# GreenleafLab/NucleoATAC

Measured on AMD Instinct MI355X. Metric: Mbp/s through occ+nuc signal pipeline, higher is better.
Workload: dtype f64

## Files before the change

nucleoatac_amd/csrc/natac_api.hip:

```cpp
#include "../../include/natac.h"
#ifndef NATAC_GNBL
#define NATAC_GNBL 2
#endif
#include "natac_kernels.hpp"
#include "natac_fft_bg.hpp"
#include "natac_occ_fast.hpp"
#include "natac_cand.hpp"
#include "natac_covsweep.hpp"
#include "natac_textz.hpp"
#include "natac_cores.hpp"
#include "natac_writer.hpp"
#include "natac_tabix.hpp"
#include "natac_pack.hpp"
#include "natac_bam.hpp"
#include "natac_bam_dev.hpp"
#include "natac_fragfile.hpp"
#include "natac_fragfile_dev.hpp"
#include "natac_fasta.hpp"
#include "natac_fuzzfit.hpp"
#include "natac_bedtab.hpp"
#include "natac_runtime.hpp"
#include "natac_pwmfit.hpp"
#include "natac_sites.hpp"
#include "natac_cellcounts.hpp"
// ... 149 lines not shown
    if (!count) return fail(NATAC_E_ARG, "count is NULL");
    int n = 0;
    hipError_t e = hipGetDeviceCount(&n);
    if (e != hipSuccess) {
        *count = 0;
        return fail(NATAC_E_HIP, "hipGetDeviceCount: %s", hipGetErrorString(e));
    }
    *count = n;
    return NATAC_OK;
}

int natac_ctx_create(int device_id, natac_ctx **out) {
    if (!out) return fail(NATAC_E_ARG, "out is NULL");
    *out = nullptr;
    int n = 0;
    HIPCHK(hipGetDeviceCount(&n));
    if (device_id < 0 || device_id >= n) return fail(NATAC_E_ARG, "device %d out of range (%d devices)", device_id, n);
    HIPCHK(hipSetDevice(device_id));
    natac_ctx *c = new natac_ctx();
    c->device = device_id;
    HIPCHK(hipGetDeviceProperties(&c->prop, device_id));
    HIPCHK(hipStreamCreateWithFlags(&c->stream, hipStreamNonBlocking));
    HIPCHK(hipEventCreate(&c->t0));
    HIPCHK(hipEventCreate(&c->t1));
    {
        const char *e = getenv("NATAC_BG_DIRECT");
        c->bg_direct = e && e[0] == '1';
        e = getenv("NATAC_BG_EXT");
        c->bg_ext = !(e && e[0] == '0');
        e = getenv("NATAC_OCC_GENERAL");
        c->occ_force_general = e && e[0] == '1';
        e = getenv("NATAC_OCC_ORDER");
        c->occ_ordered = !(e && e[0] == '0');
    }
    *out = c;
    return NATAC_OK;
}

void natac_ctx_destroy(natac_ctx *c) {
    if (!c) return;
    (void)hipSetDevice(c->device);
    (void)sync_all(c);
    prof_collect(c);
    if (c->t0) (void)hipEventDestroy(c->t0);
    if (c->t1) (void)hipEventDestroy(c->t1);
    if (c->ck_stream) (void)hipStreamDestroy(c->ck_stream);
    if (c->ck_start) (void)hipEventDestroy(c->ck_start);
    if (c->d_ck) (void)hipFree(c->d_ck);
    if (c->copy_stream) (void)hipStreamDestroy(c->copy_stream);
    if (c->stream) (void)hipStreamDestroy(c->stream);
    delete c;
}

int natac_ctx_sync(natac_ctx *c) {
    if (!c) return fail(NATAC_E_ARG, "ctx is NULL");
    HIPCHK(hipSetDevice(c->device));
    HIPCHK(sync_all(c));
    prof_collect(c);
    return NATAC_OK;
}

int natac_ctx_device_info(natac_ctx *c, char *name, size_t name_len, int *n_cu, size_t *mem_bytes) {
    if (!c) return fail(NATAC_E_ARG, "ctx is NULL");
    if (name && name_len) {
        snprintf(name, name_len, "%s (%s)", c->prop.name, c->prop.gcnArchName);
    }
// ... 234 lines not shown
        std::vector<double> tw(2 * (size_t)natac::FFT_N);
        for (int k = 0; k < natac::FFT_N; ++k) {
            const double a = 2.0 * M_PI * k / natac::FFT_N;
            tw[2 * k] = std::cos(a);
            tw[2 * k + 1] = -std::sin(a);
        }
        if (const char *e = getenv("NATAC_FAULT_TWIDDLE")) {
            int k = 0; double dlt = 0.0;
            if (sscanf(e, "%d:%lf", &k, &dlt) == 2 && k >= 0 && k < natac::FFT_N) tw[2 * (size_t)k] += dlt;
        }
        if ((rc = dev_upload(c, c->d_fft_tw, tw.data(), tw.size()))) return rc;
        HIPCHK(sync_all(c));
    }
    if (!c->fft_dirty) return NATAC_OK;
    HIPCHK(sync_all(c));
    const int npair = (c->R + 1) / 2;
    if ((rc = dev_alloc(c->d_fft_k, (size_t)npair * 2 * natac::FFT_N))) return rc;
    hipLaunchKernelGGL(natac_fft_template, dim3(npair), dim3(64), 0, c->stream, c->d_vmat, c->d_srow, c->R, c->W, c->d_fft_tw, c->d_fft_k);
    if (c->W >= natac::FFT_EXT) {
        c->d_fft_mtab.reset(); c->d_fft_swt.reset();
        const int NJ = (c->R + 3) / 4;
        if ((rc = dev_alloc(c->d_fft_mtab, (size_t)2 * NJ * 64)) || (rc = dev_alloc(c->d_fft_swt, (size_t)4 * NJ))) return rc;
        hipLaunchKernelGGL(natac_fft_edge_table_mfma, dim3((2 * NJ * 64 + 255) / 256), dim3(256), 0, c->stream, c->d_vmat, c->d_srow, c->R, c->W, NJ,
                           c->d_fft_mtab, c->d_fft_swt);
    }
    HIPCHK(hipGetLastError());
    c->fft_dirty = false;
    return NATAC_OK;
}

static int ensure_window(natac_ctx *c, PoolBuf<double> &slot, int *slotM, double *slotsd, int M, double sd, double *slotsum = nullptr) {
    if (slot && *slotM == M && *slotsd == sd) return NATAC_OK;
    HIPCHK(sync_all(c));
    std::vector<double> w((size_t)M);
    for (int i = 0; i < M; ++i) {
        double n = (double)i - (M - 1) / 2.0;
        double q = n / sd;
        w[i] = std::exp(-0.5 * (q * q));
    }
    int rc = dev_upload(c, slot, w.data(), (size_t)M);
    if (rc) return rc;
    HIPCHK(sync_all(c));
    if (slotsum) {
        double acc = 0.0;
        for (int i = 0; i < M; ++i) acc = acc + w[i];
        *slotsum = acc;
    }
    *slotM = M;
    *slotsd = sd;
    return NATAC_OK;
}

static int run_exp_bias(natac_batch *b, hipStream_t st, bool from_occ) {
    if (!b->d_bias) return NATAC_OK;
    if (from_occ && b->ebias_fresh) { b->ebias_fresh = false; return NATAC_OK; }
    b->ebias_fresh = !from_occ;
    int rc;
    if (!b->d_ebias && (rc = dev_alloc(b->d_ebias, (size_t)b->nb))) return rc;
    const int blocks = (int)std::min<long long>((b->nb + 255) / 256, 16384);
    hipLaunchKernelGGL(natac_exp_bias, dim3(blocks), dim3(256), 0, st, b->d_bias, b->d_ebias, b->nb);
    return NATAC_OK;
}

static ChunkTable make_table(natac_batch *b) {
    ChunkTable t;
    t.nc = b->nc; t.chunk_len = b->d_len; t.frag_off = b->d_frag_off; t.lpos = b->d_lpos; t.ilen = b->d_ilen;
    t.centre = b->d_centre; t.bias_off = b->d_bias_off; t.bias = b->d_bias; t.ebias = b->d_ebias; t.bias_left = b->bias_left;
    t.bias_right = b->bias_right; t.out_off = b->d_out_off; t.grid_off = b->d_grid_off;
    return t;
}
static VMatDev make_vmat(natac_ctx *c) {
    VMatDev v;
    v.mat = c->d_vmat; v.matp = c->d_vmat_pad; v.srow = c->d_srow; v.lower = c->vlower; v.upper = c->vupper; v.w = c->vw; v.R = c->R; v.W = c->W;
// ... 135 lines not shown
    delete b;
}

int natac_batch_release_outputs(natac_batch *b) {
    if (!b) return fail(NATAC_E_ARG, "batch is NULL");
    natac_ctx *c = b->ctx;
    HIPCHK(hipSetDevice(c->device));
    HIPCHK(sync_all(c));
    prof_collect(c);
    for (auto &t : b->d_track) t.reset();
    for (auto &g : b->d_grid) g.reset();
    b->d_bnum.reset(); b->d_bcov.reset(); b->d_gsum.reset(); b->d_pk_out.reset();
    b->d_pk_chunk.reset(); b->d_pk_pos.reset(); b->d_opk_vals.reset(); b->d_opk_keep.reset(); b->d_nuc_dist.reset();
    b->d_fmt_out.reset(); b->fmt_bytes = -1;
    (void)fmt_pending_wait(b);
    b->pk_cap = 0; b->pk_n = -1; b->opk_cap = 0; b->opk_n = -1;
    b->out = BatchOutputs();
    HIPCHK(hipMemsetAsync(b->d_status, 0, (size_t)b->nc * sizeof(int), c->stream));
    HIPCHK(hipStreamSynchronize(c->stream));
    return NATAC_OK;
}

int natac_batch_info(natac_batch *b, int64_t *total_bp, int64_t *total_grid, int64_t *n_frags) {
    if (!b) return fail(NATAC_E_ARG, "batch is NULL");
    if (total_bp) *total_bp = b->total_bp;
    if (total_grid) *total_grid = b->total_grid;
    if (n_frags) *n_frags = b->nf;
    return NATAC_OK;
}

static int ensure_track(natac_batch *b, int t) {
    if (b->d_track[t]) return NATAC_OK;
    return dev_alloc(b->d_track[t], (size_t)b->total_bp);
}

int natac_run_nuc(natac_batch *b, double smooth_sd) {
    if (!b) return fail(NATAC_E_ARG, "batch is NULL");
    natac_ctx *c = b->ctx;
    HIPCHK(hipSetDevice(c->device));
    int rc = ensure_srow(c);
    if (rc) return rc;
    if (!(smooth_sd > 0)) return fail(NATAC_E_ARG, "smooth_sd must be positive");
    const int M = 6 * (int)smooth_sd + 1;
    const int need_l = c->vw + ((c->vupper - 2) >> 1), need_r = c->vw + ((c->vupper - 1) >> 1) + 1;
    if (b->d_bias && (b->bias_left < need_l || b->bias_right < need_r))
        return fail(NATAC_E_ARG, "bias track must extend >= %d left / %d right of the chunk (has %d / %d)", need_l, need_r,
                    b->bias_left, b->bias_right);
    for (int i = 0; i < b->nc; ++i)
        if (b->h_len[i] < M) return fail(NATAC_E_ARG, "chunk %d shorter (%d) than the smoothing window (%d)", i, b->h_len[i], M);
    if ((rc = ensure_window(c, c->d_win_nuc, &c->win_nuc_M, &c->win_nuc_sd, M, smooth_sd, &c->win_nuc_sum))) return rc;
    const bool use_fft = fft_bg_applicable(c);
    for (int t : {NATAC_T_NUC_COV, NATAC_T_NFR_COV, NATAC_T_RAW, NATAC_T_NORM, NATAC_T_SMOOTH})
        if ((rc = ensure_track(b, t))) return rc;
    if (!use_fft && (rc = ensure_track(b, NATAC_T_BACKGROUND))) return rc;
    if (!b->d_bnum && (rc = dev_alloc(b->d_bnum, (size_t)b->total_bp))) return rc;
    if (!b->d_bcov && (rc = dev_alloc(b->d_bcov, (size_t)b->total_bp))) return rc;
    const bool fast = !use_fft && (c->W == 121 && c->vlower >= 2);
    if (use_fft) {
        if ((rc = ensure_fft(c))) return rc;
        const int TV = FFT_N - c->W + 1;
        const bool ext_ok = bg_ext_possible(c);
        const int key = -(TV + (ext_ok ? 4096 : 0));
        if (b->bgG != key) {
            if ((rc = build_tiles_bg(b, TV, ext_ok))) return rc;
            b->bgG = key;
        }
    } else if (fast) {
        const int G = choose_bg_G(b, c->W);
        if (G != b->bgG) {
            if ((rc = build_tiles(b, 64 * G, b->d_tiles_bg, &b->n_tiles_bg))) return rc;
            b->bgG = G;
        }
    }
    if (!b->d_ebias && b->d_bias && (rc = dev_alloc(b->d_ebias, (size_t)b->nb))) return rc;
    const ChunkTable ct = make_table(b);
    const VMatDev vm = make_vmat(c);
    natac_ctx::Ev ev;
    if (!b->d_ranges256 && (rc = dev_alloc(b->d_ranges256, (size_t)b->n_tiles256))) return rc;
    if ((M - 1) / 2 == 30 && !b->d_tiles1k && (rc = build_tiles(b, 1024, b->d_tiles1k, &b->n_tiles1k))) return rc;
    prof_begin(c, NATAC_K_FRAG_GATHER, ev);
    if (b->ranges256_w != c->vw) {
        hipLaunchKernelGGL(natac_tile_ranges256, dim3((b->n_tiles256 + 255) / 256), dim3(256), 0, c->stream, ct, b->d_tiles256,
                           b->n_tiles256, c->vw, b->d_ranges256);
        b->ranges256_w = c->vw;
    }
    const bool cov_mine = b->out.occ_cov_by_nuc && b->out.nuc_w == c->vw && b->out.nuc_upper == c->vupper;
    const bool cov_too = c->have_occ && c->flank == c->vw && c->occ_upper == c->vupper &&
                         (b->out.track[NATAC_T_OCC_COV] == TS_EMPTY || cov_mine);
    if (cov_too && (rc = ensure_track(b, NATAC_T_OCC_COV))) return rc;
    constexpr int GNBL = NATAC_GNBL;
    hipLaunchKernelGGL((natac_frag_gather<GNBL>), dim3(b->n_tiles256), dim3(256 / GNBL), 0, c->stream, ct, b->d_tiles256, b->d_ranges256, vm,
                       b->d_track[NATAC_T_NUC_COV], b->d_track[NATAC_T_NFR_COV], b->d_track[NATAC_T_RAW],
                       cov_too ? b->d_track[NATAC_T_OCC_COV] : nullptr);
    prof_end(c, ev);
    prof_begin(c, NATAC_K_BACKGROUND, ev);
    if ((rc = run_exp_bias(b, c->stream, false))) return rc;
    if (use_fft) {
        const size_t lds = bg_fft_lds_bytes(vm.upper);
        hipLaunchKernelGGL(natac_background_fft, dim3(b->n_tiles_bg), dim3(64), lds, c->stream, ct, b->d_tiles_bg, vm, c->d_fft_tw,
                           c->d_fft_k, b->d_track[NATAC_T_NUC_COV], b->d_track[NATAC_T_RAW], (double *)nullptr,
                           b->d_track[NATAC_T_NORM], b->d_bnum, b->d_bcov, (unsigned)b->n_tiles_bg, c->d_fft_mtab,
                           c->d_fft_swt, (c->R + 3) / 4);
    } else if (fast) {
        switch (b->bgG) {
            case 7: launch_bg<7>(b, ct, vm); break;
            case 9: launch_bg<9>(b, ct, vm); break;
            case 13: launch_bg<13>(b, ct, vm); break;
            default: launch_bg<17>(b, ct, vm); break;
        }
    } else {
        hipLaunchKernelGGL(natac_background_generic, dim3(b->n_tiles256), dim3(256), 0, c->stream, ct, b->d_tiles256, vm,
                           b->d_track[NATAC_T_NUC_COV], b->d_track[NATAC_T_RAW], b->d_track[NATAC_T_BACKGROUND],
                           b->d_track[NATAC_T_NORM], b->d_bnum, b->d_bcov);
    }
    prof_end(c, ev);
    prof_begin(c, NATAC_K_SMOOTH_NUC, ev);
    {
        const int h = (M - 1) / 2;
        if (h == 30) {
            hipLaunchKernelGGL((natac_smooth_same4<true, 30>), dim3(b->n_tiles1k), dim3(256), (size_t)8 * SM4_S(30) * sizeof(double),
                               c->stream, ct, b->d_tiles1k, c->d_win_nuc, c->win_nuc_sum, b->d_track[NATAC_T_NORM],
                               b->d_track[NATAC_T_SMOOTH]);
        } else {
            const size_t lds = ((size_t)2 * (256 + 2 * h)) * sizeof(double);
            hipLaunchKernelGGL((natac_smooth_same<true>), dim3(b->n_tiles256), dim3(256), lds, c->stream, ct, b->d_tiles256,
                               c->d_win_nuc, M, c->win_nuc_sum, b->d_track[NATAC_T_NORM], b->d_track[NATAC_T_SMOOTH]);
        }
    }
    prof_end(c, ev);
    HIPCHK(hipGetLastError());
    for (int t : {NATAC_T_NUC_COV, NATAC_T_NFR_COV, NATAC_T_RAW, NATAC_T_NORM, NATAC_T_SMOOTH}) b->out.track[t] = TS_RUN;
    b->out.track[NATAC_T_BACKGROUND] = use_fft ? TS_PENDING : TS_RUN;
    b->out.bg_gen = c->model_gen;
    b->out.nuc_w = c->vw;
    b->out.nuc_lower = c->vlower;
    b->out.nuc_upper = c->vupper;
    b->out.occ_cov_by_nuc = cov_too;
    return NATAC_OK;
}

static void launch_occ_smooth_generic(natac_batch *b, const ChunkTable &ct, const OccModelDev &om, int M, double *dst_occ, double *dst_lo,
                                      double *dst_hi) {
    natac_ctx *c = b->ctx;
    const int h = (M - 1) / 2;
    const int NB = 2 * ((h + c->step - 1) / c->step) + 2, NG = (255 + 2 * h) / c->step + 3;
    const size_t lds = ((size_t)((M + 1) & ~1) + (size_t)c->step * NB + 3 * (size_t)NG) * sizeof(double);
    hipLaunchKernelGGL(natac_occ_smooth, dim3(b->n_tiles256), dim3(256), lds, c->stream, ct, b->d_tiles256, om, c->d_win_occ, M,
                       b->d_grid[0], b->d_grid[1], b->d_grid[2], dst_occ, dst_lo, dst_hi);
}

static int occ_smooth_blocks(int h, int step) {
    if (h % step == 0) return 2 * (h / step) + 2;
    return (h + step - 1) / step + (h + step - 1) / step + 1;
}

static int ensure_block_weights(natac_ctx *c, int M, double sd, int NB) {
    if (c->d_wb_occ && c->wb_M == M && c->wb_step == c->step) return NATAC_OK;
    HIPCHK(sync_all(c));
    const int h = (M - 1) / 2, step = c->step;
    std::vector<double> w((size_t)M), wb((size_t)step * NB + step);
    for (int i = 0; i < M; ++i) {
        const double n = (double)i - (M - 1) / 2.0, q = n / sd;
        w[i] = std::exp(-0.5 * (q * q));
    }
// ... 12 lines not shown
        for (int bi = 0; bi < NB; ++bi) den = std::fma(wb[(size_t)bi * step + j], 1.0, den);
        wb[(size_t)NB * step + j] = den;
    }
    int rc = dev_upload(c, c->d_wb_occ, wb.data(), wb.size());
    if (rc) return rc;
    HIPCHK(sync_all(c));
    c->wb_M = M;
    c->wb_step = step;
    return NATAC_OK;
}

static int materialise_bg(natac_batch *b) {
    natac_ctx *c = b->ctx;
    int rc = ensure_track(b, NATAC_T_BACKGROUND);
    if (rc) return rc;
    const int blocks = (int)std::min<long long>((b->total_bp + 255) / 256, 1 << 20);
    hipLaunchKernelGGL(natac_bg_from_factors, dim3(blocks), dim3(256), 0, c->stream, b->d_bnum, b->d_track[NATAC_T_NUC_COV], b->d_bcov,
                       b->d_track[NATAC_T_BACKGROUND], b->total_bp);
    HIPCHK(hipGetLastError());
    b->out.track[NATAC_T_BACKGROUND] = TS_RUN;
    return NATAC_OK;
}

static int materialise_prefill(natac_batch *b) {
    natac_ctx *c = b->ctx;
    int rc = ensure_track(b, NATAC_T_OCC_PREFILL);
    if (rc) return rc;
    if ((rc = ensure_window(c, c->d_win_occ, &c->win_occ_M, &c->win_occ_sd, 2 * c->flank + 1, c->flank / 3.0))) return rc;
    const ChunkTable ct = make_table(b);
    const OccModelDev om = make_occ(c);
    launch_occ_smooth_generic(b, ct, om, 2 * c->flank + 1, b->d_track[NATAC_T_OCC_PREFILL], nullptr, nullptr);
    HIPCHK(hipGetLastError());
    b->out.track[NATAC_T_OCC_PREFILL] = TS_RUN;
    return NATAC_OK;
}

static int need_track(natac_batch *b, int t) {
    static const char *const names[NATAC_T_COUNT] = {"NUC_COV", "NFR_COV", "RAW", "BACKGROUND", "NORM", "SMOOTH", "OCC", "OCC_LOWER",
                                                     "OCC_UPPER", "OCC_COV", "INS", "OCC_PREFILL", "INS_SMOOTH", "CENTER_COV", "BIAS"};
    if (t < 0 || t >= NATAC_T_COUNT) return fail(NATAC_E_ARG, "bad track id %d", t);
    if (b->out.track[t] == TS_EMPTY)
        return fail(NATAC_E_STATE, "track NATAC_T_%s holds nothing: no stage has written it and natac_batch_set_track has not", names[t]);
    if (b->out.track[t] != TS_PENDING) return NATAC_OK;
    if (t == NATAC_T_OCC_PREFILL) {
        const int rc = need_occ_geometry(b, "NATAC_T_OCC_PREFILL");
        if (rc) return rc;
    }
    HIPCHK(hipSetDevice(b->ctx->device));
    return t == NATAC_T_BACKGROUND ? materialise_bg(b) : materialise_prefill(b);
}

static int occ_prepare(natac_batch *b) {
    if (!b) return fail(NATAC_E_ARG, "batch is NULL");
    natac_ctx *c = b->ctx;
    HIPCHK(hipSetDevice(c->device));
    if (!c->have_occ) return fail(NATAC_E_STATE, "natac_set_occ_model has not been called");
    const int M = 2 * c->flank + 1;
    const double sd = c->flank / 3.0;
    const int need_l = c->flank + ((c->occ_upper - 2) >> 1), need_r = c->flank + ((c->occ_upper - 1) >> 1) + 1;
    if (b->d_bias && (b->bias_left < need_l || b->bias_right < need_r))
        return fail(NATAC_E_ARG, "bias track must extend >= %d left / %d right of the chunk (has %d / %d)", need_l, need_r,
                    b->bias_left, b->bias_right);
    for (int i = 0; i < b->nc; ++i)
        if (b->h_len[i] < M) return fail(NATAC_E_ARG, "chunk %d shorter (%d) than the occupancy window (%d)", i, b->h_len[i], M);
    int rc;
    if ((rc = ensure_window(c, c->d_win_occ, &c->win_occ_M, &c->win_occ_sd, M, sd))) return rc;
    if (!b->d_grid_off || b->grid_step != c->step) {
        b->h_grid_off.assign((size_t)b->nc + 1, 0);
        for (int i = 0; i < b->nc; ++i) {
            const int nk = (b->h_len[i] > c->halfstep) ? (b->h_len[i] - c->halfstep + c->step - 1) / c->step : 0;
            b->h_grid_off[i + 1] = b->h_grid_off[i] + nk;
        }
        b->total_grid = b->h_grid_off[b->nc];
        HIPCHK(sync_all(c));
        b->out.grids = false;
        if (b->out.track[NATAC_T_OCC_PREFILL] == TS_PENDING) b->out.track[NATAC_T_OCC_PREFILL] = TS_EMPTY;
        if ((rc = dev_upload(c, b->d_grid_off, b->h_grid_off.data(), (size_t)b->nc + 1))) return rc;
        for (auto &g : b->d_grid)
            if ((rc = dev_alloc(g, (size_t)b->total_grid))) return rc;
        if ((rc = build_tiles(b, OCC_T * OCC_NP, b->d_tiles_occ, &b->n_tiles_occ, true, c->step, c->halfstep))) return rc;
        b->d_ranges_occ.reset(); b->d_order_occ.reset();
// ... 384 lines not shown
        if (dc.ok()) {
            if (mode == 1)
                hipLaunchKernelGGL(natac_cov_literal_many, dim3(NBLK, (unsigned)m), dim3(256), 0, c->stream, d_p, c->d_vmat, N, d_out);
            else if (mode == 0)
                hipLaunchKernelGGL((natac_cov_closed_many<double>), dim3((unsigned)m), dim3(256), 0, c->stream, d_p, c->d_vmat, N, d_out);
            else
                hipLaunchKernelGGL((natac_cov_closed_many<float>), dim3((unsigned)m), dim3(256), 0, c->stream, d_p, c->d_vmat, N, d_out);
            dc.launched();
        }
        dc.fetch(part.data(), d_out, (size_t)m * per);
        if ((rc = dc.sync())) return rc;
        for (int64_t k = 0; k < m; ++k) {
            double s = 0;
            for (int j = 0; j < per; ++j) s += part[(size_t)k * per + j];
            var[k0 + k] = s;
        }
    }
    std::vector<double> reads((size_t)n_cand);
    std::vector<long long> idx((size_t)n_cand);
    for (int64_t k = 0; k < n_cand; ++k) idx[(size_t)k] = b->h_out_off[cand_chunk[k]] + cand_pos[k];
    const long long *d_idx = dc.upload(idx.data(), (size_t)n_cand);
    double *d_r = dc.alloc<double>((size_t)n_cand);
    if (dc.ok()) {
        hipLaunchKernelGGL(natac_gather_f64, dim3((unsigned)((n_cand + 255) / 256)), dim3(256), 0, c->stream,
                           b->d_track[NATAC_T_NUC_COV], d_idx, (long long)n_cand, d_r);
        dc.launched();
    }
    dc.fetch(reads.data(), d_r, (size_t)n_cand);
    if ((rc = dc.finish())) return rc;
    for (int64_t k = 0; k < n_cand; ++k) var[k] = var[k] * cov_reads(reads[(size_t)k]);
    return NATAC_OK;
}

static int run_peaks_impl(natac_batch *b, const double *sig_a, const double *sig_b, bool with_stats, double min_signal, int sep,
                          int boundary, int order, const double *jitter, int64_t n_jitter, int64_t *n_cand) {
    if (!b || !jitter || !n_cand) return fail(NATAC_E_ARG, "null argument");
    natac_ctx *c = b->ctx;
    if (order < 1 || order > 255 || sep < 1 || boundary < 0) return fail(NATAC_E_ARG, "bad peak parameters");
    int maxL = 0;
    for (int i = 0; i < b->nc; ++i) maxL = std::max(maxL, b->h_len[i]);
    if (n_jitter < maxL) return fail(NATAC_E_ARG, "jitter stream (%lld) shorter than the longest chunk (%d)", (long long)n_jitter, maxL);
    HIPCHK(hipSetDevice(c->device));
    HIPCHK(sync_all(c));
    int rc;
    if (with_stats && (rc = ensure_srow(c))) return rc;
    if (!b->d_jitter || b->n_jitter < maxL) {
        if ((rc = dev_upload(c, b->d_jitter, jitter, (size_t)maxL))) return rc;
        HIPCHK(hipStreamSynchronize(c->stream));
        b->n_jitter = maxL;
    } else {
        HIPCHK(hipMemcpyAsync(b->d_jitter, jitter, (size_t)maxL * sizeof(double), hipMemcpyHostToDevice, c->stream));
        HIPCHK(hipStreamSynchronize(c->stream));
    }
    if (b->pk_order != order) {
        std::vector<long long> cap((size_t)b->nc + 1, 0);
        for (int i = 0; i < b->nc; ++i) cap[i + 1] = cap[i] + b->h_len[i] / (order + 1) + 2;
        b->slot_total = cap[b->nc];
        b->d_cap_off.reset(); b->d_slot.reset();
        if ((rc = dev_upload(c, b->d_cap_off, cap.data(), (size_t)b->nc + 1))) return rc;
        HIPCHK(hipStreamSynchronize(c->stream));
        if ((rc = dev_alloc(b->d_slot, (size_t)b->slot_total))) return rc;
        b->pk_order = order;
    }
    if (!b->d_pk_count && (rc = dev_alloc(b->d_pk_count, (size_t)b->nc))) return rc;
    if (!b->d_pk_offs && (rc = dev_alloc(b->d_pk_offs, (size_t)b->nc + 1))) return rc;
    const ChunkTable ct = make_table(b);
    const double *norm = sig_a, *sm = sig_b;
    natac_ctx::Ev ev;
    prof_begin(c, NATAC_K_CAND, ev);
    hipLaunchKernelGGL(natac_status_clear, dim3((b->nc + 255) / 256), dim3(256), 0, c->stream, b->d_status, b->nc, 2);
    {
        const int pk_cap = (std::min(PEAK_MAX, maxL / (order + 1) + 2) + 7) & ~7;
        const size_t lds_lists = (size_t)pk_cap * (sizeof(double) + sizeof(int) + 1);
        const int bt = maxL <= 4096 ? 256 : 1024;
        const int nj = (maxL + bt - 1) / bt;
        const size_t lds_reg = (size_t)((bt * nj + 2 * order + 1) & ~1) * sizeof(double) + lds_lists;
#define NATAC_PEAKS_REG(NJ, BT)                                                                                                    \
    case NJ: {                                                                                                                     \
        auto kfn = natac_peaks_chunk_reg<NJ, BT>;                                                                                  \
        if (lds_reg > 64 * 1024) HIPCHK(hipFuncSetAttribute((const void *)kfn, hipFuncAttributeMaxDynamicSharedMemorySize, (int)lds_reg)); \
        hipLaunchKernelGGL(kfn, dim3(b->nc), dim3(BT), lds_reg, c->stream, ct, norm, sm, b->d_jitter, min_signal, boundary, order, sep, \
                           pk_cap, b->d_cap_off, b->d_slot, b->d_pk_count, b->d_status);                                          \
        break;                                                                                                                     \
    }
        if (bt == 256) {
            switch (nj) {
                NATAC_PEAKS_REG(1, 256) NATAC_PEAKS_REG(2, 256) NATAC_PEAKS_REG(3, 256) NATAC_PEAKS_REG(4, 256) NATAC_PEAKS_REG(5, 256)
                NATAC_PEAKS_REG(6, 256) NATAC_PEAKS_REG(7, 256) NATAC_PEAKS_REG(8, 256) NATAC_PEAKS_REG(9, 256) NATAC_PEAKS_REG(10, 256)
                NATAC_PEAKS_REG(11, 256) NATAC_PEAKS_REG(12, 256) NATAC_PEAKS_REG(13, 256) NATAC_PEAKS_REG(14, 256)
                NATAC_PEAKS_REG(15, 256) NATAC_PEAKS_REG(16, 256)
            }
        } else if (nj <= 16 && lds_reg <= 150 * 1024) {
            switch (nj) {
                NATAC_PEAKS_REG(5, 1024) NATAC_PEAKS_REG(6, 1024) NATAC_PEAKS_REG(7, 1024) NATAC_PEAKS_REG(8, 1024) NATAC_PEAKS_REG(9, 1024)
                NATAC_PEAKS_REG(10, 1024) NATAC_PEAKS_REG(11, 1024) NATAC_PEAKS_REG(12, 1024) NATAC_PEAKS_REG(13, 1024)
                NATAC_PEAKS_REG(14, 1024) NATAC_PEAKS_REG(15, 1024) NATAC_PEAKS_REG(16, 1024)
            }
        } else {
            const int seg = 4096;
            const size_t lds = (size_t)((seg + 2 * order + 1) & ~1) * sizeof(double) + lds_lists;
            double *big_sig = nullptr;
            int *big_pos = nullptr;
            unsigned char *big_state = nullptr;
            if (maxL / (order + 1) + 2 > pk_cap) {
                if (b->d_pk_big.size() < (size_t)b->slot_total * 2 + 2 && (rc = dev_alloc(b->d_pk_big, (size_t)b->slot_total * 2 + 2)))
                    return rc;
                big_sig = b->d_pk_big;
                big_pos = (int *)(b->d_pk_big + b->slot_total);
                big_state = (unsigned char *)(big_pos + b->slot_total);
            }
            hipLaunchKernelGGL(natac_peaks_chunk, dim3(b->nc), dim3(256), lds, c->stream, ct, norm, sm, b->d_jitter, min_signal,
                               boundary, order, sep, seg, pk_cap, b->d_cap_off, b->d_slot, b->d_pk_count, b->d_status, big_sig, big_pos,
                               big_state);
        }
#undef NATAC_PEAKS_REG
    }
    hipLaunchKernelGGL(natac_scan_counts, dim3(1), dim3(1024), 0, c->stream, b->d_pk_count, b->nc, b->d_pk_offs);
    long long total = 0;
    HIPCHK(hipGetLastError());
    HIPCHK(hipMemcpyAsync(&total, b->d_pk_offs + b->nc, sizeof(long long), hipMemcpyDeviceToHost, c->stream));
    HIPCHK(hipStreamSynchronize(c->stream));
    if (total > b->pk_cap) {
        b->d_pk_chunk.reset(); b->d_pk_pos.reset(); b->d_pk_out.reset();
        b->pk_cap = 0;
        const long long cap = total + total / 4 + 16;
        if ((rc = dev_alloc(b->d_pk_chunk, (size_t)cap)) || (rc = dev_alloc(b->d_pk_pos, (size_t)cap)) ||
            (rc = dev_alloc(b->d_pk_out, (size_t)3 * cap))) {
            b->d_pk_chunk.reset(); b->d_pk_pos.reset();
            return rc;
        }
        b->pk_cap = cap;
    }
    if (total > 0) {
        hipLaunchKernelGGL(natac_compact_candidates, dim3((b->nc + 3) / 4), dim3(256), 0, c->stream, b->nc, b->d_pk_count, b->d_pk_offs,
                           b->d_cap_off, b->d_slot, b->d_pk_chunk, b->d_pk_pos);
        if (with_stats) {
            const VMatDev vm = make_vmat(c);
            launch_candidates(c, ct, vm, b->d_pk_chunk, b->d_pk_pos, total, b->d_track[NATAC_T_NUC_COV], b->d_track[NATAC_T_NORM],
                              b->out.bg_gen == c->model_gen ? b->d_bnum : nullptr, b->out.bg_gen == c->model_gen ? b->d_bcov : nullptr,
                              b->d_pk_out, b->d_pk_out + b->pk_cap, b->d_pk_out + 2 * b->pk_cap,
                              b->ranges256_w == c->vw ? b->d_tile256_first : nullptr, b->ranges256_w == c->vw ? b->d_ranges256 : nullptr);
        }
    }
    b->pk_has_stats = with_stats;
    prof_end(c, ev);
    HIPCHK(hipGetLastError());
    b->pk_n = total;
    *n_cand = total;
    return NATAC_OK;
}

int natac_run_peaks(natac_batch *b, double min_signal, int sep, int boundary, int order, const double *jitter, int64_t n_jitter,
                    int64_t *n_cand) {
    if (!b) return fail(NATAC_E_ARG, "batch is NULL");
    int rc;
    if ((rc = need_track(b, NATAC_T_SMOOTH)) || (rc = need_candidate_inputs(b)) || (rc = need_nuc_geometry(b, "natac_run_peaks"))) return rc;
    return run_peaks_impl(b, b->d_track[NATAC_T_NORM], b->d_track[NATAC_T_SMOOTH], true, min_signal, sep, boundary, order, jitter,
                          n_jitter, n_cand);
}

int natac_run_track_peaks(natac_batch *b, int track, double min_signal, int sep, int boundary, int order, const double *jitter,
                          int64_t n_jitter, int64_t *n_peaks) {
    if (!b) return fail(NATAC_E_ARG, "batch is NULL");
    if (track == NATAC_T_INS) return fail(NATAC_E_ARG, "peak search needs a float64 track");
    int rc = need_track(b, track);
    if (rc) return rc;
    return run_peaks_impl(b, b->d_track[track], nullptr, false, min_signal, sep, boundary, order, jitter, n_jitter, n_peaks);
}

int natac_run_occ_peaks(natac_batch *b, double min_occ, int sep, const double *jitter, int64_t n_jitter, int64_t *n_peaks) {
    if (!b || !n_peaks) return fail(NATAC_E_ARG, "null argument");
    int rc;
    for (int t : {NATAC_T_OCC, NATAC_T_OCC_LOWER, NATAC_T_OCC_UPPER, NATAC_T_OCC_COV}) if ((rc = need_track(b, t))) return rc;
    if ((rc = need_occ_geometry(b, "natac_run_occ_peaks"))) return rc;
    natac_ctx *c = b->ctx;
    const int U = c->occ_upper;
    if (U > 1024) return fail(NATAC_E_ARG, "upper > 1024");
    rc = run_peaks_impl(b, b->d_track[NATAC_T_OCC], nullptr, false, min_occ, sep, sep / 2, 1, jitter, n_jitter, n_peaks);
    if (rc) return rc;
    const long long n = *n_peaks;
    if (n > b->opk_cap || !b->d_opk_vals) {
        if (n > b->opk_cap) HIPCHK(sync_all(c));
        const long long cap = n > b->opk_cap ? n + n / 4 + 16 : 16;
        b->d_opk_vals.reset(); b->d_opk_keep.reset();
        b->opk_cap = 0;
        if ((rc = dev_alloc(b->d_opk_vals, (size_t)4 * cap)) || (rc = dev_alloc(b->d_opk_keep, (size_t)cap))) {
            b->d_opk_vals.reset();
            return rc;
        }
        b->opk_cap = cap;
    }
// ... 72 lines not shown
int natac_batch_download(natac_batch *b, int track, void *dst, size_t dst_bytes) {
    if (!b || !dst) return fail(NATAC_E_ARG, "null argument");
    int rc = need_track(b, track);
    if (rc) return rc;
    const size_t need = (size_t)b->total_bp * (track == NATAC_T_INS ? sizeof(int) : sizeof(double));
    if (dst_bytes != need) return fail(NATAC_E_ARG, "destination holds %zu bytes, track needs %zu", dst_bytes, need);
    HIPCHK(hipSetDevice(b->ctx->device));
    HIPCHK(hipMemcpyAsync(dst, b->d_track[track], need, hipMemcpyDeviceToHost, b->ctx->stream));
    HIPCHK(sync_all(b->ctx));
    prof_collect(b->ctx);
    return NATAC_OK;
}

int natac_batch_download_grid(natac_batch *b, int which, double *dst, size_t dst_bytes) {
    if (!b || !dst) return fail(NATAC_E_ARG, "null argument");
    if (which < 0 || which > 2) return fail(NATAC_E_ARG, "bad grid id");
    if (!b->out.grids) return fail(NATAC_E_STATE, "natac_run_occ has not run");
    const size_t need = (size_t)b->total_grid * sizeof(double);
    if (dst_bytes != need) return fail(NATAC_E_ARG, "destination holds %zu bytes, grid needs %zu", dst_bytes, need);
    HIPCHK(hipSetDevice(b->ctx->device));
    HIPCHK(hipMemcpyAsync(dst, b->d_grid[which], need, hipMemcpyDeviceToHost, b->ctx->stream));
    HIPCHK(sync_all(b->ctx));
    return NATAC_OK;
}

int natac_batch_set_track(natac_batch *b, int track, const double *vals, size_t n) {
    if (!b || !vals) return fail(NATAC_E_ARG, "null argument");
    if (track < 0 || track >= NATAC_T_COUNT || track == NATAC_T_INS) return fail(NATAC_E_ARG, "bad track id %d (float64 tracks only)", track);
    if (n != (size_t)b->total_bp) return fail(NATAC_E_ARG, "track needs %lld values, got %zu", b->total_bp, n);
    natac_ctx *c = b->ctx;
    HIPCHK(hipSetDevice(c->device));
    int rc;
    if (track == NATAC_T_NUC_COV && b->out.track[NATAC_T_BACKGROUND] == TS_PENDING && (rc = materialise_bg(b))) return rc;
    HIPCHK(sync_all(c));
    if ((rc = ensure_track(b, track))) return rc;
    HIPCHK(hipMemcpyAsync(b->d_track[track], vals, n * sizeof(double), hipMemcpyHostToDevice, c->stream));
    HIPCHK(hipStreamSynchronize(c->stream));
    b->out.track[track] = TS_HOST;
    if (track == NATAC_T_OCC_COV) b->out.occ_cov_by_nuc = false;
    return NATAC_OK;
}

int natac_batch_status(natac_batch *b, int32_t *dst, size_t dst_bytes) {
    if (!b || !dst) return fail(NATAC_E_ARG, "null argument");
    if (dst_bytes != (size_t)b->nc * sizeof(int)) return fail(NATAC_E_ARG, "status buffer must hold n_chunks int32");
    HIPCHK(hipSetDevice(b->ctx->device));
    HIPCHK(hipMemcpyAsync(dst, b->d_status, dst_bytes, hipMemcpyDeviceToHost, b->ctx->stream));
    HIPCHK(sync_all(b->ctx));
    return NATAC_OK;
}

int natac_batch_track_ptr(natac_batch *b, int track, void **dptr) {
    if (!b || !dptr) return fail(NATAC_E_ARG, "null argument");
    if (track < 0 || track >= NATAC_T_COUNT) return fail(NATAC_E_ARG, "bad track id");
    *dptr = nullptr;
    if (b->out.track[track] == TS_EMPTY) return NATAC_OK;
    int rc = need_track(b, track);
    if (rc) return rc;
    *dptr = b->d_track[track];
    return NATAC_OK;
}


int natac_host_alloc(size_t bytes, void **out) {
    if (!out) return fail(NATAC_E_ARG, "out is NULL");
    *out = nullptr;
// ... 27 lines not shown
```

nucleoatac_amd/csrc/natac_kernels.hpp:

```cpp
#pragma once
#include <hip/hip_runtime.h>
#include <stdint.h>

#include <type_traits>

namespace natac {

constexpr int WAVE = 64;

struct ChunkTable {
    int nc;
    const int *chunk_len;
    const long long *frag_off;
    const int *lpos;
    const int *ilen;
    const int *centre;
    const long long *bias_off;
    const double *bias;
    const double *ebias;
    int bias_left, bias_right;
    const long long *out_off;
    const long long *grid_off;
};

// ... 1657 lines not shown
            const int g = x0 + 256 * it + threadIdx.x;
            v[it] = 0.0;
            if (pkf & (1u << it)) v[it] = smooth ? norm[ob + g] + smooth[ob + g] : norm[ob + g];
        }
        unsigned long long bal[16];
#pragma unroll
        for (int it = 0; it < 16; ++it) {
            const int g = x0 + 256 * it + threadIdx.x;
            if (v[it] != v[it]) v[it] = fillv;
            const bool pk = (pkf & (1u << it)) && (v[it] >= min_signal) && (g >= boundary) && (g < L - boundary);
            bal[it] = __ballot(pk);
            if (lane == 0) row_cnt[it * 4 + wave] = __popcll(bal[it]);
        }
        __syncthreads();
#pragma unroll
        for (int it = 0; it < 16; ++it) {
            int off = n;
#pragma unroll
            for (int w = 0; w < 4; ++w) {
                const int cw = row_cnt[it * 4 + w];
                off += (w < wave) ? cw : 0;
                n += cw;
            }
            if ((bal[it] >> lane) & 1ull) {
                const int i = off + __popcll(bal[it] & ((1ull << lane) - 1ull));
                if (i < pk_cap) { pos[i] = x0 + 256 * it + threadIdx.x; sig[i] = v[it]; state[i] = 0; }
            }
        }
    }
    __syncthreads();
    peaks_thin_and_write(n, pk_cap, sep, sig, pos, state, wave_cnt, cand_slot + cap_off[chunk], count + chunk, status + chunk);
}

template <int NJ, int BT>
__global__ void __launch_bounds__(BT) natac_peaks_chunk_reg(ChunkTable ct, const double *__restrict__ norm,
                                                               const double *__restrict__ smooth, const double *__restrict__ jitter,
                                                               double min_signal, int boundary, int order, int sep, int pk_cap,
                                                               const long long *__restrict__ cap_off, int *__restrict__ cand_slot,
                                                               int *__restrict__ count, int *__restrict__ status) {
    extern __shared__ __attribute__((aligned(16))) double smem[];
    constexpr int NW = BT / 64;
    __shared__ double red[NW];
    __shared__ int wave_cnt[16];
    __shared__ int row_cnt[NW * NJ];
    const int ysn = (BT * NJ + 2 * order + 1) & ~1;
    double *ys = smem;
    double *sig = ys + ysn;
    int *pos = (int *)(sig + pk_cap);
    unsigned char *state = (unsigned char *)(pos + pk_cap);
    const int chunk = blockIdx.x;
    const int L = ct.chunk_len[chunk];
    const long long ob = ct.out_off[chunk];
    const int wave = threadIdx.x >> 6, lane = threadIdx.x & 63;
    double v[NJ], jt[NJ];
#pragma unroll
    for (int j = 0; j < NJ; ++j) {
        const int g = threadIdx.x + BT * j;
        v[j] = __builtin_nan("");
        jt[j] = 0.0;
        if (g < L) {
            v[j] = smooth ? norm[ob + g] + smooth[ob + g] : norm[ob + g];
            jt[j] = jitter[g];
        }
    }
    double mn = __builtin_inf();
#pragma unroll
    for (int j = 0; j < NJ; ++j)
        if (v[j] == v[j]) mn = fmin(mn, v[j]);
    mn = wave_min(mn);
    if (lane == 0) red[wave] = mn;
    __syncthreads();
    double fillv = red[0];
#pragma unroll
    for (int w = 1; w < NW; ++w) fillv = fmin(fillv, red[w]);
    if (fillv == __builtin_inf()) {
        if (threadIdx.x == 0) count[chunk] = 0;
        return;
    }
#pragma unroll
    for (int j = 0; j < NJ; ++j) {
        const int g = threadIdx.x + BT * j;
        if (v[j] != v[j]) v[j] = fillv;
        if (g < L) {
            const double y = v[j] * (1 + jt[j]);
            ys[order + g] = y;
            if (g == 0)
                for (int u = 0; u < order; ++u) ys[u] = y;
            if (g == L - 1)
                for (int u = 0; u < order; ++u) ys[order + L + u] = y;
        }
    }
    __syncthreads();
    unsigned long long bal[NJ];
    {
        const int region = pk_cap * (int)(sizeof(double) + sizeof(int) + 1);
        const int stride = (region / NW) & ~7;
// ... 464 lines not shown
```

nucleoatac_amd/csrc/natac_runtime.hpp:

```cpp
#pragma once
#include "../../include/natac.h"
#include "natac_textz.hpp"

#include <algorithm>
#include <cstdarg>
#include <cstdio>
#include <cstdlib>
#include <map>
#include <mutex>
#include <string>
#include <unordered_map>
#include <utility>
#include <vector>

static thread_local std::string g_err;

static int fail(int code, const char *fmt, ...) {
    char buf[512];
    va_list ap;
    va_start(ap, fmt);
    vsnprintf(buf, sizeof buf, fmt, ap);
    va_end(ap);
    g_err = buf;
    return code;
// ... 30 lines not shown
        return e;
    }
    T *get() const { return p_; }
    operator T *() const { return p_; }
    size_t size() const { return n_; }

  private:
    T *p_ = nullptr;
    size_t n_ = 0;
};

template <class T>
static int dev_alloc(PoolBuf<T> &buf, size_t n) {
    HIPCHK(buf.alloc(n));
    return NATAC_OK;
}

struct natac_ctx {
    int device = 0;
    hipStream_t stream = nullptr;
    hipStream_t copy_stream = nullptr;
    hipDeviceProp_t prop;
    PoolBuf<double> d_vmat, d_vmat_pad, d_srow, d_sizes;
    PoolBuf<double> d_lrt;
    long long lrt_gen = -1;
    PoolBuf<double> d_ctab;
    long long ctab_gen = -1;
    int vlower = 0, vupper = 0, vw = 0, R = 0, W = 0, sizes_upper = 0;
    bool have_vmat = false, have_sizes = false, srow_dirty = true;
    bool vmat_zero = false, srow_zero = false;
    long long model_gen = 0;
    PoolBuf<double> d_fft_tw, d_fft_k;
    PoolBuf<double> d_fft_mtab, d_fft_swt;
    bool bg_ext = true;
    bool fft_dirty = true, bg_direct = false, occ_ordered = true, occ_zero_nfr = false;
    std::vector<double> h_sizes;
    PoolBuf<double> d_nucp, d_nfrp, d_alphas;
    int occ_upper = 0, n_alpha = 0, step = 0, halfstep = 0, flank = 0;
    double cutoff = 0;
    bool have_occ = false;
    int occ_zero_flags = 0;
    PoolBuf<double> d_occ_q4, d_occ_rho;
    int occ_nm = 0;
    bool occ_fast_ok = false, occ_force_general = false, occ_rn16 = false;
    double occ_b_floor = 0;
    PoolBuf<double> d_win_nuc, d_win_occ;
    PoolBuf<double> d_wb_occ;
    int wb_M = 0, wb_step = 0;
    int win_nuc_M = 0, win_occ_M = 0;
    double win_nuc_sd = -1, win_occ_sd = -1;
    double win_nuc_sum = 0, win_occ_sum = 0;
    bool profiling = false;
    struct Ev { int k; hipEvent_t a, b; hipStream_t st; };
    std::vector<Ev> pending;
    double prof_ms[NATAC_K_COUNT] = {0};
    int64_t prof_n[NATAC_K_COUNT] = {0};
    hipEvent_t t0 = nullptr, t1 = nullptr;
    hipStream_t ck_stream = nullptr;
    hipEvent_t ck_start = nullptr;
    long long *d_ck = nullptr;
    int ck_cap = 0;
    bool ck_active = false;
    struct Iv { int k; float t0, t1; };
    std::vector<Iv> ck_iv;
    PoolBuf<natac_text::P10> d_p10;
    PoolBuf<natac_deflate::CrcTables> d_crc;
};

enum TrackState : unsigned char { TS_EMPTY = 0, TS_PENDING, TS_RUN , TS_HOST  };
struct BatchOutputs {
    TrackState track[NATAC_T_COUNT] = {};
    bool grids = false;
    long long bg_gen = -1;
    int nuc_w = -1, nuc_lower = -1, nuc_upper = -1;
    bool occ_cov_by_nuc = false;
    int occ_step = -1, occ_half = -1, occ_flank = -1, occ_upper = -1;
};

struct natac_batch {
    natac_ctx *ctx = nullptr;
    int nc = 0;
    long long nf = 0, nb = 0, total_bp = 0, total_grid = 0;
    int bias_left = 0, bias_right = 0;
    std::vector<int> h_len;
    std::vector<long long> h_out_off, h_grid_off;
    PoolBuf<int> d_len, d_lpos, d_ilen, d_centre, d_status;
    PoolBuf<long long> d_frag_off, d_bias_off, d_out_off, d_grid_off;
    PoolBuf<double> d_bias, d_ebias;
    PoolBuf<unsigned long long> d_occ_minkey;
    PoolBuf<int> d_occ_nan;
    int n_tiles_os = 0, os_width = 0;
    PoolBuf<int2> d_tiles_os, d_tiles1k;
    int n_tiles1k = 0;
    PoolBuf<int2> d_tiles256, d_tiles_bg, d_tiles_occ, d_ranges_occ, d_ranges256;
    PoolBuf<long long> d_tile256_first;
    PoolBuf<int> d_order_occ;
    int ranges256_w = -1;
    int ranges_occ_key[3] = {-1, -1, -1};
    int n_tiles256 = 0, n_tiles_bg = 0, n_tiles_occ = 0, bgG = 0;
    int grid_step = 0, grid_half = 0;
    PoolBuf<long long> d_blk_off;
    long long total_blocks = 0;
    PoolBuf<double> d_gsum;
    PoolBuf<int2> d_tiles_gs;
    int n_tiles_gs = 0, gs_Q = -1;
    PoolBuf<int> d_defer;
    PoolBuf<double> d_opk_vals, d_nuc_dist;
    PoolBuf<int> d_opk_keep;
// ... 244 lines not shown
```

Baseline: 3469.

## Defer nucleosome smoothing and fuse it into the peak-calling kernel

When smoothing half-width is 30 and every chunk is at most 4096 bp, the separate nucleosome smoothing kernel is deferred and marked pending. The peak-calling kernel then computes the smoothed track in LDS from the normalized signal, writes it out, and uses it directly. This removes one kernel launch and one global read of the smoothed track. NaN-aware denominators use precomputed prefix and suffix window sums plus ballot bitmasks. The risks are extra LDS and register pressure in the peaks kernel, and a slower fallback path when the NaN pattern is irregular.

Result: faster. 3516 (median of 6 runs) (+1.3%).

```diff
diff --git a/nucleoatac_amd/csrc/natac_api.hip b/nucleoatac_amd/csrc/natac_api.hip
--- a/nucleoatac_amd/csrc/natac_api.hip
+++ b/nucleoatac_amd/csrc/natac_api.hip
@@ -205,6 +205,8 @@
         c->occ_force_general = e && e[0] == '1';
         e = getenv("NATAC_OCC_ORDER");
         c->occ_ordered = !(e && e[0] == '0');
+        e = getenv("NATAC_SMOOTH_FUSED");
+        c->smooth_fused = !(e && e[0] == '0');
     }
     *out = c;
     return NATAC_OK;
@@ -505,13 +507,19 @@
 static int ensure_window(natac_ctx *c, PoolBuf<double> &slot, int *slotM, double *slotsd, int M, double sd, double *slotsum = nullptr) {
     if (slot && *slotM == M && *slotsd == sd) return NATAC_OK;
     HIPCHK(sync_all(c));
-    std::vector<double> w((size_t)M);
+    std::vector<double> w((size_t)3 * M);
     for (int i = 0; i < M; ++i) {
         double n = (double)i - (M - 1) / 2.0;
         double q = n / sd;
         w[i] = std::exp(-0.5 * (q * q));
     }
-    int rc = dev_upload(c, slot, w.data(), (size_t)M);
+    for (int m = 0; m < M; ++m) w[M + m] = (m ? w[M + m - 1] : 0.0) + w[m];
+    for (int k = 0; k < M; ++k) {
+        double acc = 0.0;
+        for (int i = k; i < M; ++i) acc = acc + w[i];
+        w[2 * M + k] = acc;
+    }
+    int rc = dev_upload(c, slot, w.data(), (size_t)3 * M);
     if (rc) return rc;
     HIPCHK(sync_all(c));
     if (slotsum) {
@@ -713,6 +721,27 @@
 static int ensure_track(natac_batch *b, int t) {
     if (b->d_track[t]) return NATAC_OK;
     return dev_alloc(b->d_track[t], (size_t)b->total_bp);
+}
+
+static void launch_nuc_smooth(natac_batch *b, const ChunkTable &ct, int M) {
+    natac_ctx *c = b->ctx;
+    const int h = (M - 1) / 2;
+    if (h == 30) {
+        hipLaunchKernelGGL((natac_smooth_same4<true, 30>), dim3(b->n_tiles1k), dim3(256), (size_t)8 * SM4_S(30) * sizeof(double),
+                           c->stream, ct, b->d_tiles1k, c->d_win_nuc, c->win_nuc_sum, b->d_track[NATAC_T_NORM],
+                           b->d_track[NATAC_T_SMOOTH]);
+    } else {
+        const size_t lds = ((size_t)2 * (256 + 2 * h)) * sizeof(double);
+        hipLaunchKernelGGL((natac_smooth_same<true>), dim3(b->n_tiles256), dim3(256), lds, c->stream, ct, b->d_tiles256,
+                           c->d_win_nuc, M, c->win_nuc_sum, b->d_track[NATAC_T_NORM], b->d_track[NATAC_T_SMOOTH]);
+    }
+}
+
+static bool peaks_can_smooth(const natac_batch *b, int M) {
+    if (!b->ctx->smooth_fused || (M - 1) / 2 != PK_SM_H) return false;
+    for (int i = 0; i < b->nc; ++i)
+        if (b->h_len[i] > 4096) return false;
+    return true;
 }
 
 int natac_run_nuc(natac_batch *b, double smooth_sd) {
@@ -758,7 +787,8 @@
     const VMatDev vm = make_vmat(c);
     natac_ctx::Ev ev;
     if (!b->d_ranges256 && (rc = dev_alloc(b->d_ranges256, (size_t)b->n_tiles256))) return rc;
-    if ((M - 1) / 2 == 30 && !b->d_tiles1k && (rc = build_tiles(b, 1024, b->d_tiles1k, &b->n_tiles1k))) return rc;
+    const bool smooth_later = peaks_can_smooth(b, M);
+    if (!smooth_later && (M - 1) / 2 == 30 && !b->d_tiles1k && (rc = build_tiles(b, 1024, b->d_tiles1k, &b->n_tiles1k))) return rc;
     prof_begin(c, NATAC_K_FRAG_GATHER, ev);
     if (b->ranges256_w != c->vw) {
         hipLaunchKernelGGL(natac_tile_ranges256, dim3((b->n_tiles256 + 255) / 256), dim3(256), 0, c->stream, ct, b->d_tiles256,
@@ -795,22 +825,16 @@
                            b->d_track[NATAC_T_NORM], b->d_bnum, b->d_bcov);
     }
     prof_end(c, ev);
-    prof_begin(c, NATAC_K_SMOOTH_NUC, ev);
-    {
-        const int h = (M - 1) / 2;
-        if (h == 30) {
-            hipLaunchKernelGGL((natac_smooth_same4<true, 30>), dim3(b->n_tiles1k), dim3(256), (size_t)8 * SM4_S(30) * sizeof(double),
-                               c->stream, ct, b->d_tiles1k, c->d_win_nuc, c->win_nuc_sum, b->d_track[NATAC_T_NORM],
-                               b->d_track[NATAC_T_SMOOTH]);
-        } else {
-            const size_t lds = ((size_t)2 * (256 + 2 * h)) * sizeof(double);
-            hipLaunchKernelGGL((natac_smooth_same<true>), dim3(b->n_tiles256), dim3(256), lds, c->stream, ct, b->d_tiles256,
-                               c->d_win_nuc, M, c->win_nuc_sum, b->d_track[NATAC_T_NORM], b->d_track[NATAC_T_SMOOTH]);
-        }
-    }
-    prof_end(c, ev);
+    if (!smooth_later) {
+        prof_begin(c, NATAC_K_SMOOTH_NUC, ev);
+        launch_nuc_smooth(b, ct, M);
+        prof_end(c, ev);
+    }
     HIPCHK(hipGetLastError());
     for (int t : {NATAC_T_NUC_COV, NATAC_T_NFR_COV, NATAC_T_RAW, NATAC_T_NORM, NATAC_T_SMOOTH}) b->out.track[t] = TS_RUN;
+    if (smooth_later) b->out.track[NATAC_T_SMOOTH] = TS_PENDING;
+    b->out.smooth_M = M;
+    b->out.smooth_sd = smooth_sd;
     b->out.track[NATAC_T_BACKGROUND] = use_fft ? TS_PENDING : TS_RUN;
     b->out.bg_gen = c->model_gen;
     b->out.nuc_w = c->vw;
@@ -889,6 +913,21 @@
     launch_occ_smooth_generic(b, ct, om, 2 * c->flank + 1, b->d_track[NATAC_T_OCC_PREFILL], nullptr, nullptr);
     HIPCHK(hipGetLastError());
     b->out.track[NATAC_T_OCC_PREFILL] = TS_RUN;
+    return NATAC_OK;
+}
+
+static int materialise_smooth(natac_batch *b) {
+    natac_ctx *c = b->ctx;
+    int rc;
+    if ((rc = ensure_window(c, c->d_win_nuc, &c->win_nuc_M, &c->win_nuc_sd, b->out.smooth_M, b->out.smooth_sd, &c->win_nuc_sum))) return rc;
+    if ((b->out.smooth_M - 1) / 2 == 30 && !b->d_tiles1k && (rc = build_tiles(b, 1024, b->d_tiles1k, &b->n_tiles1k))) return rc;
+    const ChunkTable ct = make_table(b);
+    natac_ctx::Ev ev;
+    prof_begin(c, NATAC_K_SMOOTH_NUC, ev);
+    launch_nuc_smooth(b, ct, b->out.smooth_M);
+    prof_end(c, ev);
+    HIPCHK(hipGetLastError());
+    b->out.track[NATAC_T_SMOOTH] = TS_RUN;
     return NATAC_OK;
 }
 
@@ -904,6 +943,7 @@
         if (rc) return rc;
     }
     HIPCHK(hipSetDevice(b->ctx->device));
+    if (t == NATAC_T_SMOOTH) return materialise_smooth(b);
     return t == NATAC_T_BACKGROUND ? materialise_bg(b) : materialise_prefill(b);
 }
 
@@ -1354,8 +1394,18 @@
     return NATAC_OK;
 }
 
+static int peaks_list_cap(int maxL, int order) { return (std::min(PEAK_MAX, maxL / (order + 1) + 2) + 7) & ~7; }
+
+static bool peaks_smooth_arm(const natac_batch *b, int order) {
+    if (order < 1 || order > 255) return false;
+    int maxL = 0;
+    for (int i = 0; i < b->nc; ++i) maxL = std::max(maxL, b->h_len[i]);
+    const int region = peaks_list_cap(maxL, order) * (int)(sizeof(double) + sizeof(int) + 1), nj = (maxL + 255) / 256;
+    return ((region / 4) & ~7) >= nj * 8;
+}
+
 static int run_peaks_impl(natac_batch *b, const double *sig_a, const double *sig_b, bool with_stats, double min_signal, int sep,
-                          int boundary, int order, const double *jitter, int64_t n_jitter, int64_t *n_cand) {
+                          int boundary, int order, const double *jitter, int64_t n_jitter, int64_t *n_cand, bool form_smooth = false) {
     if (!b || !jitter || !n_cand) return fail(NATAC_E_ARG, "null argument");
     natac_ctx *c = b->ctx;
     if (order < 1 || order > 255 || sep < 1 || boundary < 0) return fail(NATAC_E_ARG, "bad peak parameters");
@@ -1386,23 +1436,27 @@
     }
     if (!b->d_pk_count && (rc = dev_alloc(b->d_pk_count, (size_t)b->nc))) return rc;
     if (!b->d_pk_offs && (rc = dev_alloc(b->d_pk_offs, (size_t)b->nc + 1))) return rc;
+    if (form_smooth &&
+        (rc = ensure_window(c, c->d_win_nuc, &c->win_nuc_M, &c->win_nuc_sd, b->out.smooth_M, b->out.smooth_sd, &c->win_nuc_sum))) return rc;
     const ChunkTable ct = make_table(b);
     const double *norm = sig_a, *sm = sig_b;
     natac_ctx::Ev ev;
     prof_begin(c, NATAC_K_CAND, ev);
     hipLaunchKernelGGL(natac_status_clear, dim3((b->nc + 255) / 256), dim3(256), 0, c->stream, b->d_status, b->nc, 2);
     {
-        const int pk_cap = (std::min(PEAK_MAX, maxL / (order + 1) + 2) + 7) & ~7;
+        const int pk_cap = peaks_list_cap(maxL, order);
         const size_t lds_lists = (size_t)pk_cap * (sizeof(double) + sizeof(int) + 1);
         const int bt = maxL <= 4096 ? 256 : 1024;
         const int nj = (maxL + bt - 1) / bt;
-        const size_t lds_reg = (size_t)((bt * nj + 2 * order + 1) & ~1) * sizeof(double) + lds_lists;
+        const size_t lds_reg = (size_t)peaks_reg_ysn(bt * nj, order, form_smooth) * sizeof(double) + lds_lists;
+        double *sm_out = form_smooth ? b->d_track[NATAC_T_SMOOTH].get() : nullptr;
+        if (form_smooth) sm = nullptr;
 #define NATAC_PEAKS_REG(NJ, BT)                                                                                                    \
     case NJ: {                                                                                                                     \
-        auto kfn = natac_peaks_chunk_reg<NJ, BT>;                                                                                  \
+        auto kfn = form_smooth ? natac_peaks_chunk_reg<NJ, BT, BT == 256> : natac_peaks_chunk_reg<NJ, BT, false>;                  \
         if (lds_reg > 64 * 1024) HIPCHK(hipFuncSetAttribute((const void *)kfn, hipFuncAttributeMaxDynamicSharedMemorySize, (int)lds_reg)); \
         hipLaunchKernelGGL(kfn, dim3(b->nc), dim3(BT), lds_reg, c->stream, ct, norm, sm, b->d_jitter, min_signal, boundary, order, sep, \
-                           pk_cap, b->d_cap_off, b->d_slot, b->d_pk_count, b->d_status);                                          \
+                           pk_cap, b->d_cap_off, b->d_slot, b->d_pk_count, b->d_status, c->d_win_nuc, c->win_nuc_sum, sm_out);     \
         break;                                                                                                                     \
     }
         if (bt == 256) {
@@ -1440,6 +1494,7 @@
     hipLaunchKernelGGL(natac_scan_counts, dim3(1), dim3(1024), 0, c->stream, b->d_pk_count, b->nc, b->d_pk_offs);
     long long total = 0;
     HIPCHK(hipGetLastError());
+    if (form_smooth) b->out.track[NATAC_T_SMOOTH] = TS_RUN;
     HIPCHK(hipMemcpyAsync(&total, b->d_pk_offs + b->nc, sizeof(long long), hipMemcpyDeviceToHost, c->stream));
     HIPCHK(hipStreamSynchronize(c->stream));
     if (total > b->pk_cap) {
@@ -1476,9 +1531,11 @@
                     int64_t *n_cand) {
     if (!b) return fail(NATAC_E_ARG, "batch is NULL");
     int rc;
-    if ((rc = need_track(b, NATAC_T_SMOOTH)) || (rc = need_candidate_inputs(b)) || (rc = need_nuc_geometry(b, "natac_run_peaks"))) return rc;
+    const bool form_smooth = b->out.track[NATAC_T_SMOOTH] == TS_PENDING && peaks_smooth_arm(b, order);
+    if ((!form_smooth && (rc = need_track(b, NATAC_T_SMOOTH))) || (rc = need_candidate_inputs(b)) ||
+        (rc = need_nuc_geometry(b, "natac_run_peaks"))) return rc;
     return run_peaks_impl(b, b->d_track[NATAC_T_NORM], b->d_track[NATAC_T_SMOOTH], true, min_signal, sep, boundary, order, jitter,
-                          n_jitter, n_cand);
+                          n_jitter, n_cand, form_smooth);
 }
 
 int natac_run_track_peaks(natac_batch *b, int track, double min_signal, int sep, int boundary, int order, const double *jitter,
@@ -1617,6 +1674,7 @@
     HIPCHK(hipSetDevice(c->device));
     int rc;
     if (track == NATAC_T_NUC_COV && b->out.track[NATAC_T_BACKGROUND] == TS_PENDING && (rc = materialise_bg(b))) return rc;
+    if (track == NATAC_T_NORM && b->out.track[NATAC_T_SMOOTH] == TS_PENDING && (rc = materialise_smooth(b))) return rc;
     HIPCHK(sync_all(c));
     if ((rc = ensure_track(b, track))) return rc;
     HIPCHK(hipMemcpyAsync(b->d_track[track], vals, n * sizeof(double), hipMemcpyHostToDevice, c->stream));
diff --git a/nucleoatac_amd/csrc/natac_kernels.hpp b/nucleoatac_amd/csrc/natac_kernels.hpp
--- a/nucleoatac_amd/csrc/natac_kernels.hpp
+++ b/nucleoatac_amd/csrc/natac_kernels.hpp
@@ -1713,18 +1713,26 @@
     peaks_thin_and_write(n, pk_cap, sep, sig, pos, state, wave_cnt, cand_slot + cap_off[chunk], count + chunk, status + chunk);
 }
 
-template <int NJ, int BT>
+constexpr int PK_SM_H = 30;
+
+__host__ __device__ constexpr int peaks_reg_ysn(int bt_nj, int order, bool smooth) {
+    return (bt_nj + ((smooth && 2 * PK_SM_H > 2 * order + 1) ? 2 * PK_SM_H : 2 * order + 1)) & ~1;
+}
+
+template <int NJ, int BT, bool SMOOTH = false>
 __global__ void __launch_bounds__(BT) natac_peaks_chunk_reg(ChunkTable ct, const double *__restrict__ norm,
                                                                const double *__restrict__ smooth, const double *__restrict__ jitter,
                                                                double min_signal, int boundary, int order, int sep, int pk_cap,
                                                                const long long *__restrict__ cap_off, int *__restrict__ cand_slot,
-                                                               int *__restrict__ count, int *__restrict__ status) {
+                                                               int *__restrict__ count, int *__restrict__ status,
+                                                               const double *__restrict__ win, double win_sum,
+                                                               double *__restrict__ smooth_out) {
     extern __shared__ __attribute__((aligned(16))) double smem[];
     constexpr int NW = BT / 64;
     __shared__ double red[NW];
     __shared__ int wave_cnt[16];
     __shared__ int row_cnt[NW * NJ];
-    const int ysn = (BT * NJ + 2 * order + 1) & ~1;
+    const int ysn = peaks_reg_ysn(BT * NJ, order, SMOOTH);
     double *ys = smem;
     double *sig = ys + ysn;
     int *pos = (int *)(sig + pk_cap);
@@ -1734,6 +1742,88 @@
     const long long ob = ct.out_off[chunk];
     const int wave = threadIdx.x >> 6, lane = threadIdx.x & 63;
     double v[NJ], jt[NJ];
+    if constexpr (SMOOTH) {
+        constexpr int H = PK_SM_H, M = 2 * H + 1;
+        static_assert(BT >= 2 * H && M < 64, "the halo is zeroed by one pass of the workgroup; a window's validity bits fit one word");
+        __shared__ unsigned long long okb[NW * NJ + 2];
+        double *xs = smem;
+#pragma unroll
+        for (int j = 0; j < NJ; ++j) {
+            const int g = threadIdx.x + BT * j;
+            double x = __builtin_nan("");
+            if (g < L) x = norm[ob + g];
+            v[j] = x;
+            const bool okv = x == x;
+            xs[H + g] = okv ? (x < 0 ? 0.0 : x) : 0.0;
+            const unsigned long long m = __ballot(okv);
+            if (lane == 0) okb[1 + NW * j + wave] = m;
+        }
+        if (threadIdx.x < 2 * H) xs[threadIdx.x < H ? threadIdx.x : BT * NJ + threadIdx.x] = 0.0;
+        if (threadIdx.x == 0) { okb[0] = 0ull; okb[NW * NJ + 1] = 0ull; }
+        __syncthreads();
+        const int g0 = threadIdx.x * NJ;
+        double num[NJ];
+#pragma unroll
+        for (int o = 0; o < NJ; ++o) num[o] = 0.0;
+        if (g0 < L) {
+#pragma unroll
+            for (int kk = 0; kk < 2 * H + NJ; ++kk) {
+                const int k = 2 * H + NJ - 1 - kk;
+                const double r = xs[g0 + k];
+#pragma unroll
+                for (int o = 0; o < NJ; ++o) {
+                    const int n = o + 2 * H - k;
+                    if (n >= 0 && n < M) num[o] = fma(win[n], r, num[o]);
+                }
+            }
+        }
+        __syncthreads();
+        if (g0 < L) {
+#pragma unroll
+            for (int o = 0; o < NJ; ++o) xs[g0 + o] = num[o];
+        }
+        __syncthreads();
+#pragma unroll
+        for (int j = 0; j < NJ; ++j) {
+            const int g = threadIdx.x + BT * j;
+            const bool in = g < L;
+            jt[j] = 0.0;
+            if (in) jt[j] = jitter[g];
+            double den = win_sum;
+            const int iw = NW * j + wave;
+            constexpr unsigned long long HM = (1ull << H) - 1ull;
+            const bool clean = (okb[iw] >> (64 - H)) == HM && okb[iw + 1] == ~0ull && (okb[iw + 2] & HM) == HM;
+            if (__ballot(!clean) != 0ull) {
+                constexpr unsigned long long FULL = (1ull << M) - 1ull;
+                const int p = g - H + 64, i = p >> 6, sh = p & 63;
+                unsigned long long f = okb[i] >> sh;
+                if (sh) f |= okb[i + 1] << (64 - sh);
+                f &= FULL;
+                bool generic = false;
+                if (in && f != FULL) {
+                    const int lo = __builtin_ctzll(f | (1ull << M)), hi = __builtin_clzll(f | 1ull) - (64 - M);
+                    if (f == 0ull) den = 0.0;
+                    else if (f == ((FULL >> lo) << lo)) den = win[M + 2 * H - lo];
+                    else if (f == (FULL >> hi)) den = win[2 * M + hi];
+                    else generic = true;
+                }
+                if (__ballot(generic) != 0ull) {
+                    double d = 0.0;
+#pragma unroll 8
+                    for (int n = 0; n < M; ++n) {
+                        const double wv = win[n];
+                        if ((f >> (2 * H - n)) & 1ull) d = fma(wv, 1.0, d);
+                    }
+                    if (generic) den = d;
+                }
+            }
+            if (in) {
+                const double s = (den == 0.0) ? __builtin_nan("") : xs[g] / den;
+                smooth_out[ob + g] = s;
+                v[j] += s;
+            }
+        }
+    } else {
 #pragma unroll
     for (int j = 0; j < NJ; ++j) {
         const int g = threadIdx.x + BT * j;
@@ -1743,6 +1833,7 @@
             v[j] = smooth ? norm[ob + g] + smooth[ob + g] : norm[ob + g];
             jt[j] = jitter[g];
         }
+    }
     }
     double mn = __builtin_inf();
 #pragma unroll
diff --git a/nucleoatac_amd/csrc/natac_runtime.hpp b/nucleoatac_amd/csrc/natac_runtime.hpp
--- a/nucleoatac_amd/csrc/natac_runtime.hpp
+++ b/nucleoatac_amd/csrc/natac_runtime.hpp
@@ -86,6 +86,7 @@
     long long model_gen = 0;
     PoolBuf<double> d_fft_tw, d_fft_k;
     PoolBuf<double> d_fft_mtab, d_fft_swt;
+    bool smooth_fused = true;
     bool bg_ext = true;
     bool fft_dirty = true, bg_direct = false, occ_ordered = true, occ_zero_nfr = false;
     std::vector<double> h_sizes;
@@ -128,6 +129,8 @@
     long long bg_gen = -1;
     int nuc_w = -1, nuc_lower = -1, nuc_upper = -1;
     bool occ_cov_by_nuc = false;
+    int smooth_M = 0;
+    double smooth_sd = 0;
     int occ_step = -1, occ_half = -1, occ_flank = -1, occ_upper = -1;
 };
 
```
